# hatoo/rene

Measured on AMD Instinct MI355X. Metric: Mrays/s, higher is better.
Workload: dtype f32

## Files before the change

### include/rene_hip.h

```cpp
#ifndef RENE_HIP_H
#define RENE_HIP_H

#include <stddef.h>
#include <stdint.h>

#ifdef __cplusplus
extern "C" {
#endif

#define RENE_ABI_VERSION 7u

typedef enum rene_status {
  RENE_OK = 0,
  RENE_ERR_INVALID_ARGUMENT = -1,
  RENE_ERR_INVALID_SCENE = -2,
  RENE_ERR_DEVICE = -3,
  RENE_ERR_UNSUPPORTED = -4,
  RENE_ERR_OUT_OF_MEMORY = -5,
  RENE_ERR_IO = -6,
  RENE_ERR_PARSE = -7
} rene_status;


enum { RENE_SHAPE_TRIANGLE = 0, RENE_SHAPE_SPHERE = 1 };
// ... 356 lines not shown

int rene_emitter_pdf(rene_ctx* ctx, size_t n, const float* origins, const float* directions, float* out);

int rene_pcg_probe(int device, uint32_t seed, uint32_t n, uint32_t* out);

int rene_frame_stream_probe(rene_ctx* ctx, uint32_t first_frame, uint32_t n_frames, float* out);

int rene_load_chains(rene_ctx* ctx, const float* chains, size_t n_floats, uint32_t first_frame, uint32_t n_frames,
                     const uint32_t* tile_frames, size_t n_tiles);

#define RENE_COMM_ID_BYTES 128
int rene_comm_unique_id(uint8_t id[RENE_COMM_ID_BYTES]);
int rene_comm_init(rene_ctx* ctx, int n_ranks, int rank, const uint8_t id[RENE_COMM_ID_BYTES]);
int rene_comm_init_all(rene_ctx** ctxs, int n);
int rene_comm_group_begin(void);
int rene_comm_group_end(void);
int rene_reduce(rene_ctx* ctx, int root);
int rene_gather_tiles(rene_ctx* ctx, int root);

void rene_destroy(rene_ctx* ctx);

int rene_scene_pack_info(const rene_scene_desc* scene, rene_pack_info* out);

int rene_plan_memory(const rene_scene_desc* scene, const rene_opts* opts, rene_memory_plan* out);

const char* rene_last_error(void);
uint32_t rene_abi_version(void);


void rene_to_rgb8(const float* sums, size_t n_floats, uint32_t n_samples, uint8_t* out);
void rene_to_aov8(const float* sums, size_t n_floats, uint32_t n_samples, int is_normal, uint8_t* out);
void rene_frame_seeds(uint32_t master_seed, uint32_t first_frame, uint32_t n, uint32_t* out);


typedef struct rene_scene rene_scene;

int rene_scene_load_pbrt(const char* path, rene_scene** out);
int rene_scene_parse_pbrt(const char* text, const char* base_dir, rene_scene** out);
const rene_scene_desc* rene_scene_get_desc(const rene_scene* scene);
const char* rene_scene_film_filename(const rene_scene* scene);
void rene_scene_free(rene_scene* scene);

#ifdef __cplusplus
}
#endif
#endif
// ... 1 lines not shown
```

### rene_amd/abi.py

```python
from __future__ import annotations

import ctypes as C

ABI_VERSION = 7
COMM_ID_BYTES = 128
DEFAULT_SEED = 0x52454E45
TILE_SIZE = 32
FRAME_STREAM_DEPTHS = 50

SHAPE_TRIANGLE, SHAPE_SPHERE = 0, 1
(MATERIAL_NONE, MATERIAL_MATTE, MATERIAL_GLASS, MATERIAL_SUBSTRATE, MATERIAL_METAL,
 MATERIAL_MIRROR, MATERIAL_UBER, MATERIAL_PLASTIC) = range(8)
TEXTURE_SOLID, TEXTURE_CHECKERBOARD, TEXTURE_IMAGEMAP, TEXTURE_SCALE = range(4)
AREA_LIGHT_NULL, AREA_LIGHT_DIFFUSE = 0, 1
LIGHT_DISTANT = 0
INTEGRATOR_PATH, INTEGRATOR_VOLPATH = 0, 1
LAYER_RADIANCE, LAYER_NORMAL, LAYER_ALBEDO = 0, 1, 2
FLAG_COUNTERS, FLAG_NO_AOV, FLAG_FORCE_BVH, FLAG_SINGLE_LEVEL, FLAG_NO_RESTART, FLAG_DYNAMIC_FIRST, FLAG_WAVEFRONT = 1, 2, 4, 8, 16, 32, 64
FLAG_OVERLAP = 128
FLAG_FP16_PAYLOAD = 256
FLAG_FRAME_GROUPS = 1 << 9
FEAT_SMALL = 64
SHARD_TILES, SHARD_FRAMES = 0, 1

STATUS_NAMES = {
    0: "RENE_OK", -1: "RENE_ERR_INVALID_ARGUMENT", -2: "RENE_ERR_INVALID_SCENE",
    -3: "RENE_ERR_DEVICE", -4: "RENE_ERR_UNSUPPORTED", -5: "RENE_ERR_OUT_OF_MEMORY",
    -6: "RENE_ERR_IO", -7: "RENE_ERR_PARSE",
}

f32, u32, i32, u64 = C.c_float, C.c_uint32, C.c_int32, C.c_uint64


class Vertex(C.Structure):
    _fields_ = [("position", f32 * 3), ("normal", f32 * 3), ("uv", f32 * 2)]


class Mesh(C.Structure):
    _fields_ = [("vertices", C.POINTER(Vertex)), ("indices", C.POINTER(u32)),
                ("n_vertices", u32), ("n_indices", u32)]


class Instance(C.Structure):
    _fields_ = [("shape", u32), ("mesh_index", i32), ("material_index", u32),
# ... 167 lines not shown

class Hit(C.Structure):
    _fields_ = [("t", f32), ("u", f32), ("v", f32), ("instance", u32), ("primitive", u32)]


def algorithmic_bytes(stats) -> int:
    g = (lambda k: stats[k]) if isinstance(stats, dict) else (lambda k: getattr(stats, k))
    n_ray = g("rays_closest") + g("rays_shadow") + g("rays_emitter")
    return (64 * n_ray + 64 * g("node_visits") + 48 * g("prim_tests") + 144 * g("hits")
            + 128 * g("bounces") + 32 * g("adds"))


EXPORTED_SYMBOLS = [
    "rene_create", "rene_render", "rene_sync", "rene_download", "rene_reset", "rene_tune", "rene_framebuffer",
    "rene_get_stats", "rene_denoise_params_default", "rene_denoise", "rene_denoise_tiles", "rene_download_denoised", "rene_denoised_buffer",
    "rene_noise_params_default", "rene_estimate_noise", "rene_download_noise_tiles", "rene_noise_combine", "rene_noise_frames_needed",
    "rene_set_active_tiles", "rene_tile_frames", "rene_download_mean", "rene_noise_select_tiles",
    "rene_robust_params_default", "rene_resolve_robust", "rene_download_robust", "rene_download_robust_tiles", "rene_robust_combine",
    "rene_denoise_robust_params_default", "rene_denoise_robust", "rene_denoise_tiles_robust",
    "rene_denoise_shard_bytes", "rene_denoise_shard_prepare", "rene_denoise_shard_buffer", "rene_download_denoise_shard",
    "rene_denoise_place_shard", "rene_denoise_placed", "rene_gather_denoise",
    "rene_feature_params_default", "rene_feature_channels", "rene_export_features", "rene_features_buffer", "rene_download_features", "rene_trace", "rene_ray_dump", "rene_trace_queue", "rene_bsdf_eval", "rene_medium_eval", "rene_emitter_pdf", "rene_pcg_probe", "rene_frame_stream_probe", "rene_load_chains",
    "rene_comm_unique_id", "rene_comm_init", "rene_comm_init_all", "rene_comm_group_begin", "rene_comm_group_end",
    "rene_reduce", "rene_gather_tiles", "rene_destroy", "rene_scene_pack_info", "rene_plan_memory", "rene_last_error", "rene_abi_version",
    "rene_to_rgb8", "rene_to_aov8", "rene_frame_seeds",
    "rene_scene_load_pbrt", "rene_scene_parse_pbrt", "rene_scene_get_desc",
    "rene_scene_film_filename", "rene_scene_free",
]
```

### rene_amd/api.py

```python
from __future__ import annotations

import ctypes as C
import os
import subprocess

import numpy as np

from . import abi

_CSRC = os.path.join(os.path.dirname(os.path.abspath(__file__)), "csrc")
LIB_PATH = os.path.join(_CSRC, os.environ.get("RENE_HIP_LIB", "librene_hip.so"))
_LIB = None


class ReneError(RuntimeError):
    def __init__(self, code: int, message: str):
        super().__init__(f"{abi.STATUS_NAMES.get(code, code)}: {message}")
        self.code = code


def build(force: bool = False) -> str:
    args = ["make", "-C", _CSRC, "-j4"]
    if force:
        args.append("-B")
# ... 60 lines not shown
    L.rene_feature_params_default.argtypes = [C.POINTER(abi.FeatureParams)]
    L.rene_feature_params_default.restype = None
    L.rene_feature_channels.argtypes = [u32]
    L.rene_feature_channels.restype = u32
    L.rene_export_features.argtypes = [vp, C.POINTER(abi.FeatureParams), vp, C.c_size_t]
    L.rene_features_buffer.argtypes = [vp, C.POINTER(vp), C.POINTER(C.c_size_t)]
    L.rene_download_features.argtypes = [vp, vp, C.c_size_t]
    L.rene_trace.argtypes = [vp, i32, C.c_size_t, vp, vp, C.c_float, C.c_float, vp]
    L.rene_bsdf_eval.argtypes = [vp, u32, C.c_size_t, vp, vp, vp, vp, vp, vp]
    L.rene_medium_eval.argtypes = [vp, u32, C.c_size_t, vp, vp, vp, vp, vp, vp]
    L.rene_emitter_pdf.argtypes = [vp, C.c_size_t, vp, vp, vp]
    L.rene_pcg_probe.argtypes = [i32, u32, u32, vp]
    L.rene_frame_stream_probe.argtypes = [vp, u32, u32, vp]
    L.rene_load_chains.argtypes = [vp, vp, C.c_size_t, u32, u32, vp, C.c_size_t]
    L.rene_ray_dump.argtypes = [vp, u32, u32, C.c_size_t, vp, C.POINTER(C.c_uint64)]
    L.rene_trace_queue.argtypes = [vp, C.c_size_t, vp, vp, i32, u32, u32, u32, u32, vp, C.POINTER(C.c_float), vp]
    L.rene_comm_unique_id.argtypes = [vp]
    L.rene_comm_init.argtypes = [vp, i32, i32, vp]
    L.rene_comm_init_all.argtypes = [C.POINTER(vp), i32]
    L.rene_reduce.argtypes = [vp, i32]
    L.rene_gather_tiles.argtypes = [vp, i32]
    L.rene_destroy.argtypes = [vp]
    L.rene_scene_pack_info.argtypes = [C.POINTER(abi.SceneDesc), C.POINTER(abi.PackInfo)]
    L.rene_plan_memory.argtypes = [C.POINTER(abi.SceneDesc), C.POINTER(abi.Opts), C.POINTER(abi.MemoryPlan)]
    L.rene_destroy.restype = None
    L.rene_last_error.restype = C.c_char_p
    L.rene_abi_version.restype = u32
    L.rene_to_rgb8.argtypes = [vp, C.c_size_t, u32, vp]
    L.rene_to_rgb8.restype = None
    L.rene_to_aov8.argtypes = [vp, C.c_size_t, u32, i32, vp]
    L.rene_to_aov8.restype = None
    L.rene_frame_seeds.argtypes = [u32, u32, u32, vp]
    L.rene_frame_seeds.restype = None
    L.rene_scene_load_pbrt.argtypes = [C.c_char_p, C.POINTER(vp)]
    L.rene_scene_parse_pbrt.argtypes = [C.c_char_p, C.c_char_p, C.POINTER(vp)]
    L.rene_scene_get_desc.argtypes = [vp]
    L.rene_scene_get_desc.restype = C.POINTER(abi.SceneDesc)
    L.rene_scene_film_filename.argtypes = [vp]
    L.rene_scene_film_filename.restype = C.c_char_p
    L.rene_scene_free.argtypes = [vp]
    L.rene_scene_free.restype = None
    if L.rene_abi_version() != abi.ABI_VERSION:
        raise ReneError(-1, "librene_hip.so ABI version differs from rene_amd.abi")
    _LIB = L
    return L

# ... 567 lines not shown

Renderer.bsdf_eval = _bsdf_eval


def _medium_eval(self, medium_index: int, rd, t_max, wo, wi, seeds) -> np.ndarray:
    a = [np.ascontiguousarray(v, dtype=np.float32) for v in (rd, t_max, wo, wi)]
    sd = np.ascontiguousarray(seeds, dtype=np.uint32)
    out = np.zeros((sd.size, 16), np.float32)
    p = lambda x: x.ctypes.data_as(C.c_void_p)
    _check(lib().rene_medium_eval(self._h, medium_index, sd.size, p(a[0]), p(a[1]), p(a[2]), p(a[3]), p(sd), p(out)))
    return out


Renderer.medium_eval = _medium_eval


def pack_info(scene) -> abi.PackInfo:
    packed = scene if hasattr(scene, "byref") else scene.to_desc()
    info = abi.PackInfo()
    _check(lib().rene_scene_pack_info(packed.byref(), C.byref(info)))
    return info


def plan_memory(scene, seed: int = abi.DEFAULT_SEED, device: int = 0, flags: int = 0, shard_mode: int = abi.SHARD_TILES,
                shard_rank: int = 0, shard_count: int = 1, framebuffer_ptr: int | None = None, stream_ptr: int | None = None) -> dict:
    packed = scene if hasattr(scene, "byref") else scene.to_desc()
    o = abi.Opts()
    o.struct_size = C.sizeof(abi.Opts)
    o.seed, o.device, o.flags = seed & 0xFFFFFFFF, device, flags
    o.shard_mode, o.shard_rank, o.shard_count = shard_mode, shard_rank, shard_count
    o.framebuffer = framebuffer_ptr
    o.stream = stream_ptr
    plan = abi.MemoryPlan()
    _check(lib().rene_plan_memory(packed.byref(), C.byref(o), C.byref(plan)))
    return plan.as_dict()


def to_rgb8(sums: np.ndarray, n_samples: int) -> np.ndarray:
    a = np.ascontiguousarray(sums, dtype=np.float32)
    out = np.empty(a.shape, dtype=np.uint8)
    lib().rene_to_rgb8(a.ctypes.data_as(C.c_void_p), a.size, n_samples, out.ctypes.data_as(C.c_void_p))
    return out


def to_aov8(sums: np.ndarray, n_samples: int, is_normal: bool) -> np.ndarray:
    a = np.ascontiguousarray(sums, dtype=np.float32)
# ... 10 lines not shown
```

### rene_amd/csrc/device_code.inc

```
#include <hip/hip_runtime.h>

#include <algorithm>
#include <cstdio>
#include <cstdlib>
#include <mutex>
#include <unordered_map>

#include "device_math.h"
#include "device_scene.h"
#include "kernels.h"

namespace rene {

constexpr int BLOCK = 256;

struct HitRec {
  float t, u, v;
  uint32_t slot;
};

struct LaneCounters {
  uint32_t closest = 0, shadow = 0, emitter = 0, paths = 0, hits = 0, adds = 0, nodes = 0, prims = 0;
};

// ... 209 lines not shown
  if (shift == 0u) {
    for (uint32_t i = threadIdx.x; i < P.n_frames; i += BLOCK) T2[i] = frame_seed(P.seed_state0, P.first_frame + i * P.frame_stride);
    return;
  }
  const uint32_t B = 1u << shift, n1 = (P.n_frames + B - 1u) >> shift;
  __attribute__((address_space(3))) uint32_t* T1 = T2 + 2u * B;
  for (uint32_t j = threadIdx.x; j < B; j += BLOCK) {
    uint32_t m, a;
    lcg_pow(j * P.frame_stride, m, a);
    T2[2u * j] = m;
    T2[2u * j + 1u] = a;
  }
  for (uint32_t k = threadIdx.x; k < n1; k += BLOCK) T1[k] = frame_state(P.seed_state0, P.first_frame + (k << shift) * P.frame_stride);
}
RENE_DEV uint32_t launch_seed(const RenderParams& P, const uint32_t* lds_base, uint32_t i) {
  if (P.seed_tab == SEED_TAB_NONE) return frame_seed(P.seed_state0, P.first_frame + i * P.frame_stride);
  const uint32_t shift = P.seed_tab >> 24;
  const __attribute__((address_space(3))) uint32_t* T2 = (const __attribute__((address_space(3))) uint32_t*)lds_base + (P.seed_tab & 0xffffffu);
  if (shift == 0u) return T2[i];
  const uint32_t B = 1u << shift, j = i & (B - 1u);
  return pcg_output(T2[2u * B + (i >> shift)] * T2[2u * j] + T2[2u * j + 1u]);
}

template <bool ANY, bool SPHERES, bool COUNT, bool ITEMS_LDS = false>
RENE_DEV HitRec traverse_small(const Accel& A, const Sphere* spheres, f3 o, f3 d, float tmin, float tmax,
                               LaneCounters& lc, lds_ptr lds_items = nullptr) {
  float best_t = __uint_as_float(__float_as_uint(tmax) + 1u), best_s = 0.0f, best_r = 0.0f;
  uint32_t best_item = 0xffffffffu;
  const uint32_t n = A.n_items;
  typedef const __attribute__((address_space(4))) float16v* item_ptr;
  item_ptr base = (item_ptr)(const void*)A.items;
  auto test_item = [&](const float16v q, const uint32_t k) {
    const float kind = q[12];
    if (COUNT) lc.prims++;
    if (SPHERES && kind == SMALL_KIND_BALL) {
      f3 oc = mk3(o.x - q[0], o.y - q[1], o.z - q[2]);
      float a = length_squared(d);
      float half_b = dot(oc, d);
      float c = length_squared(oc) - q[3];
      float disc = half_b * half_b - a * c;
      if (disc >= 0.0f) {
        float sq = fast_sqrt(disc);
        float inv_a = fast_rcp(a);
        float root0 = (-half_b - sq) * inv_a;
        float root1 = (-half_b + sq) * inv_a;
        float r = -1.0f;
        if (root0 >= tmin && root0 < best_t) r = root0;
        else if (root1 >= tmin && root1 < best_t) r = root1;
        if (r >= tmin && r < best_t) {
          best_t = r;
// ... 44 lines not shown
      }
      const uint32_t open_face = __float_as_uint(q[14]);
      bool use_in = t_in >= tmin, dead = false;
      if (open_face != 0u) {
        const float t_open = open_face == 1u ? t0 : t1;
        use_in = use_in && t_in != t_open;
        dead = !use_in && t_out == t_open;
      }
      const float t = use_in ? t_in : t_out;
      if (t_in <= t_out && !dead && t >= tmin && t < best_t) {
        best_t = t;
        best_item = k;
      }
      return;
    }
    const float n_o = o.x * q[0] + (o.y * q[1] + o.z * q[2]);
    const float n_d = d.x * q[0] + (d.y * q[1] + d.z * q[2]);
    float t = (q[3] - n_o) * __builtin_amdgcn_rcpf(n_d);
    f3 P = mk3(fmaf(t, d.x, o.x), fmaf(t, d.y, o.y), fmaf(t, d.z, o.z));
    const float sr_x = fmaf(P.x, q[4], fmaf(P.y, q[6], P.z * q[8])) + q[10];
    const float sr_y = fmaf(P.x, q[5], fmaf(P.y, q[7], P.z * q[9])) + q[11];
    const float lim_x = fmaf(-kind, sr_y, 1.0f - sr_x), lim_y = fmaf(-kind, sr_x, 1.0f - sr_y);
    bool accept = fminf(fminf(sr_x, sr_y), fminf(lim_x, lim_y)) >= 0.0f && t >= tmin && t < best_t;
    if (accept) {
      best_t = t;
      best_s = sr_x;
      best_r = sr_y;
      best_item = k;
    }
  };
  for (uint32_t k = 0; k < n; ++k) test_item(base[k], k);
  HitRec h;
  h.t = best_t;
  h.u = 0.0f;
  h.v = 0.0f;
  h.slot = 0xffffffffu;
  if (ANY && best_item != 0xffffffffu) {
    h.slot = 0u;
    return h;
  }
  if (best_item != 0xffffffffu) {
    float4 m = ITEMS_LDS ? lds4(lds_items + 16u * best_item + 12u) : ldg4(A.items[best_item].q + 12);
    if (m.x == SMALL_KIND_BOX) {
      float4 b0, b1, b2;
      if (ITEMS_LDS) {
        lds_ptr bq = lds_items + 16u * best_item;
// ... 885 lines not shown
template <bool SPHERES>
RENE_DEV float emitter_pdf_lds(const SceneView& S, const SmallLds& T, const HitRec& h, f3 ro, f3 rd) {
  if (h.slot == 0xffffffffu) return 0.0f;
  lds_ptr q = T.emit + SMALL_EMIT_FLOATS * h.slot;
  const float4 a = lds4(q), b = lds4(q + 4), c = lds4(q + 8), pr = lds4(q + 12);
  const float primitive_count = q[16];
  uint32_t sidx = __float_as_uint(c.w);
  if (SPHERES && sidx != 0xffffffffu) {
    const lds_ptr sq = T.spheres + 24u * sidx;
    const float4 m0 = lds4(sq), m1 = lds4(sq + 4), m2 = lds4(sq + 8);
    const float m[12] = {m0.x, m0.y, m0.z, m0.w, m1.x, m1.y, m1.z, m1.w, m2.x, m2.y, m2.z, m2.w};
    float radius = (fabsf(m[0]) + fabsf(m[4]) + fabsf(m[8])) / 3.0f;
    f3 center = mk3(m[9], m[10], m[11]);
    float cos_theta_max = fast_sqrt(fmaxf(1.0f - qdiv(radius * radius, length_squared(center - ro)), 0.0f));
    float solid_angle = 2.0f * kPi * (1.0f - cos_theta_max);
    return fast_rcp(solid_angle);
  }
  f3 p0 = mk3(a.x, a.y, a.z), e1 = mk3(a.w, b.x, b.y), e2 = mk3(b.z, b.w, c.x);
  f3 hit_pos = p0 + h.u * e1 + h.v * e2;
  float distance_squared = length_squared(ro - hit_pos);
  float cosine = fabsf(dot(normalize(rd), mk3(pr.x, pr.y, pr.z)));
  return qdiv(qdiv(distance_squared, cosine * pr.w), primitive_count);
}
template <bool SPHERES>
RENE_DEV f3 emit_sample_lds(const SmallLds& T, uint32_t obj, Pcg& rng) {
  lds_ptr e = T.eobj + 16u * obj;
  const float4 head = lds4(e);
  if (SPHERES && __float_as_uint(head.x) == 1u) {
    f3 v = normalize(random_in_unit_sphere(rng));
    const float4 m0 = lds4(e + 4), m1 = lds4(e + 8), m2 = lds4(e + 12);
    const float m[12] = {m0.x, m0.y, m0.z, m0.w, m1.x, m1.y, m1.z, m1.w, m2.x, m2.y, m2.z, m2.w};
    return aff_point(m, v);
  }
  uint32_t p = umod(pcg_u32(rng), __float_as_uint(head.z));
  lds_ptr q = T.etri + 12u * (__float_as_uint(head.y) + p);
  const float4 a = lds4(q), b = lds4(q + 4), c = lds4(q + 8);
  float r = pcg_f32(rng);
  float s = pcg_f32(rng);
  if (r + s > 1.0f) {
    r = 1.0f - r;
    s = 1.0f - s;
  }
  return mk3(a.x, a.y, a.z) * (1.0f - r - s) + mk3(a.w, b.x, b.y) * r + mk3(b.z, b.w, c.x) * s;
}

struct MediumRec {
// ... 383 lines not shown
  V.shade = global_ptr<PrimShade>(karg_u64_at<RENE_SKARG(shade)>(KB, tick));
  V.emit_pdf = global_ptr<EmitPdf>(karg_u64_at<RENE_SKARG(emit_pdf)>(KB, tick));
  V.insts = global_ptr<Inst>(karg_u64_at<RENE_SKARG(insts)>(KB, tick));
  V.emit_objects = global_ptr<EmitObject>(karg_u64_at<RENE_SKARG(emit_objects)>(KB, tick));
  V.emit_tris = global_ptr<EmitTri>(karg_u64_at<RENE_SKARG(emit_tris)>(KB, tick));
  V.materials = global_ptr<Material>(karg_u64_at<RENE_SKARG(materials)>(KB, tick));
  V.textures = global_ptr<Texture>(karg_u64_at<RENE_SKARG(textures)>(KB, tick));
  V.lights = global_ptr<Light>(karg_u64_at<RENE_SKARG(lights)>(KB, tick));
  V.images = global_ptr<ImageRef>(karg_u64_at<RENE_SKARG(images)>(KB, tick));
  V.image_pool = global_ptr<float>(karg_u64_at<RENE_SKARG(image_pool)>(KB, tick));
  V.uni = global_ptr<struct Uniforms>(karg_u64_at<RENE_SKARG(uni)>(KB, tick));
  return V;
}

#ifdef RENE_NO_FRAME_STREAM_TABLE
constexpr bool kFrameStreamTable = false;
#else
constexpr bool kFrameStreamTable = true;
#endif
#ifndef RENE_FRAME_STREAM_LOAD_EARLY
#define RENE_FRAME_STREAM_LOAD_EARLY 0
#endif
constexpr bool frame_stream_feat(uint32_t feat) { return kFrameStreamTable && (feat & FEAT_SMALL) && !(feat & (FEAT_VOLPATH | FEAT_SPHERES)) && lobe_kinds(feat) == 0; }
RENE_DEV float4 frame_stream_load(const float* table, uint32_t launch_frame, uint32_t depth) {
  const uint32_t off = ((launch_frame << FRAME_STREAM_STRIDE_LOG2) + depth) << 4;
  const lds_v4 e = *(const __attribute__((address_space(1))) lds_v4*)((const __attribute__((address_space(1))) char*)table + off);
  return make_float4(e.x, e.y, e.z, e.w);
}
template <bool SPHERES>
RENE_DEV void frame_stream_row(const SceneView& S, uint32_t seed, float4* row) {
  Pcg fw = pcg_new(seed);
  for (uint32_t depth = 0; depth < FRAME_STREAM_DEPTHS; ++depth) {
    f3 on_light = splat(0.0f);
    uint32_t light = 0u;
    if (S.emit_object_len > 0) {
      if (pcg_f32(fw) > 0.5f) {
        uint32_t obj = umod(pcg_u32(fw), S.emit_object_len);
        on_light = emit_sample<SPHERES>(S, obj, fw);
        light = 0x80000000u;
      }
    }
    float rr_coin = 0.0f;
    if (depth > 12) rr_coin = pcg_f32(fw);
    row[depth] = make_float4(on_light.x, on_light.y, on_light.z, __uint_as_float(__float_as_uint(rr_coin) | light));
  }
}

#ifndef RENE_REGEN_MIN
#define RENE_REGEN_MIN 1
#endif
template <uint32_t FEAT, int MAXL, bool COUNT, bool AOV>
#ifndef RENE_SMALL_GEN1_PLAIN_WAVES
#define RENE_SMALL_GEN1_PLAIN_WAVES 1
#endif
#ifndef RENE_SMALL_GEN1_WAVES
#define RENE_SMALL_GEN1_WAVES 1
#endif
__global__ void __launch_bounds__(BLOCK, (FEAT & FEAT_SMALL) && !(FEAT & FEAT_VOLPATH) ? (!(FEAT & FEAT_GENERAL_BSDF) ? RENE_SMALL_MATTE_WAVES : (MAXL == 1 ? ((FEAT & FEAT_TEXTURES) ? RENE_SMALL_GEN1_WAVES : RENE_SMALL_GEN1_PLAIN_WAVES) : 1)) : 1) render_kernel(SceneView S, RenderParams P) {
  constexpr bool SPHERES = (FEAT & FEAT_SPHERES) != 0;
  constexpr uint32_t GENERAL = lobe_kinds(FEAT);
  constexpr bool SMALL = (FEAT & FEAT_SMALL) != 0;
  constexpr bool VOL = (FEAT & FEAT_VOLPATH) != 0;
  extern __shared__ uint32_t s_stack[];
  uint32_t* stack = s_stack + threadIdx.x;
  constexpr bool LDS = SMALL && !VOL;
  constexpr bool FWTAB = frame_stream_feat(FEAT);
  SmallLds T{};
  if constexpr (LDS) {
    small_lds_fill(S, s_stack);
    T = small_lds(S, s_stack);
  }
  seed_tables_fill(P, s_stack);
  __syncthreads();

  LaneCounters lc;
  const uint32_t W = S.width, H = S.height;
  const float tmin = 0.001f, tmax = 100000.0f;

  uint32_t ver = 0, pxy = 0, frame = 0, frame_end = 0;
  const karg_ptr KB = (karg_ptr)__builtin_amdgcn_kernarg_segment_ptr();
  auto rec_offset = [&]() { return pixel_record(KB, pxy & 0x3fffu, H - 1 - ((pxy >> 14) & 0x3fffu), pxy >> 28) * 4; };
  bool waiting = false;
  f3 acc0 = splat(0.0f), acc1 = splat(0.0f), acc2 = splat(0.0f);
  bool active = false, done = false;
  f3 ro = splat(0.0f), rd = splat(0.0f), color = splat(0.0f);
  Pcg rng{0}, fw{0};
  int depth = 0;
  uint32_t medium_index = 0;

  const size_t layer_stride = (size_t)(P.n_work >> CHAINS_LOG2) * 4;
  uint32_t batch_next = 0, batch_ll = 0;
  bool exhausted = false;
  first_batch(P, KB, batch_next, batch_ll);
  clock_probe(P, false);

  uint32_t iter = 0;
  uint32_t ln_active = 0, ln_wait = 0, ln_idle = 0, ln_start = 0, st_switch = 0, st_poll = 0;
  for (;; ++iter) {
    bool finished = !active && !waiting && ver != 0u && frame == frame_end;
    if (finished) {
      float* p = reinterpret_cast<float*>(karg_u64<RENE_KARG(framebuffer)>(KB)) + rec_offset();
      item_commit<AOV>(ver, p, layer_stride, acc0, acc1, acc2);
      ver = 0u;
    }
    if (COUNT && __any(finished)) st_switch++;
    bool need = !done && ver == 0u;
    bool fresh = false;
    if (__any(need)) {
      if ((batch_ll & 0xffffu) == 0u && !exhausted) exhausted = !batch_refill(KB, batch_next, batch_ll);
      unsigned long long mask = __ballot(need);
      uint32_t rank = (uint32_t)__popcll(mask & ((1ull << lane_id()) - 1ull));
// ... 62 lines not shown
      if (n_start < RENE_REGEN_MIN && __any(active)) start_now = false;
    }
    if (start_now) {
      const uint32_t seed = launch_seed(P, s_stack, frame);
      frame += CHAINS;
      const uint32_t px = pxy & 0x3fffu, py = (pxy >> 14) & 0x3fffu;
      rng = pcg_new((py * W + px) ^ seed);
      if constexpr (!FWTAB) fw = pcg_new(seed);
      float u = qdiv((float)px + pcg_f32(rng), (float)(W - 1));
      float v = qdiv((float)py + pcg_f32(rng), (float)(H - 1));
      cfloat_ptr cam = (cfloat_ptr)(const void*)S.uni;
      f3 origin = camera_origin(cam);
      f3 target = m4_point(cam + 16, mk3(u * 2.0f - 1.0f, v * 2.0f - 1.0f, 1.0f));
      target = m4_point(cam, target);
      ro = origin;
      rd = normalize(target - origin);
      color = splat(1.0f);
      depth = 0;
      medium_index = 0;
      active = true;
    }

    if (active) {
      lc.closest++;
      float4 fwe = make_float4(0.0f, 0.0f, 0.0f, 0.0f);
      if constexpr (FWTAB && RENE_FRAME_STREAM_LOAD_EARLY) fwe = frame_stream_load(P.frame_stream, frame - CHAINS, (uint32_t)depth);
      HitRec h = trace_accel<SMALL, false, SPHERES, COUNT, LDS>(S.main, S.spheres, ro, rd, tmin, tmax, stack, lc, T.items_main);
      if (h.slot == 0xffffffffu) {
        f3 bg = splat(0.0f);
        if (FEAT & FEAT_BACKGROUND) {
          uv2 uv = sphere_uv(normalize(m4_vector(S.uni->bg_matrix, rd)));
          bg = mk3(S.uni->bg_color[0], S.uni->bg_color[1], S.uni->bg_color[2]) * background_tex<FEAT>(S, uv);
        }
        acc0 = acc0 + color * bg;
        lc.adds++;
        active = false;
      } else if (VOL) {
        lc.hits++;
        Surface sf = shade_hit<SPHERES>(S, h, ro, rd);
        const Inst& inst = S.insts[sf.instance];
        f3 wo = -normalize(rd);
        f3 normal = normalize(sf.normal);
        f3 position = sf.position;
        MediumRec medium = load_medium(S, medium_index);
        bool scattered = false;
        if (medium.type != RENE_MEDIUM_VACUUM) {
          SampledMedium sm = medium_sample(medium, ro, rd, h.t, rng);
          color = color * sm.tr;
          scattered = sm.sampled;
          if (scattered) ro = sm.position;
        }
// ... 121 lines not shown
        }
        if (depth == 0) {
          if (AOV) {
            acc1 = acc1 + normal;
            acc2 = acc2 + material_albedo<FEAT>(L, inst, sf.uv);
          }
          lc.adds += 2;
        }
        if (FEAT & FEAT_LIGHTS) {
          for (uint32_t li = 0; li < L.lights_len; ++li) {
            float4 ld = ldg4(L.lights[li].dir), lL = ldg4(L.lights[li].L);
            f3 target = position + mk3(ld.x, ld.y, ld.z);
            f3 wi = normalize(target - position);
            lc.shadow++;
            HitRec sh = trace_accel<SMALL, true, SPHERES, COUNT, LDS>(S.main, S.spheres, position, wi, tmin, 1e5f, stack, lc, T.items_main);
            if (sh.slot == 0xffffffffu) {
              f3 f = bsdf_f<MAXL, GENERAL>(bsdf, wo, wi);
              acc0 = acc0 + color * f * fabsf(dot(wi, normal)) * mk3(lL.x, lL.y, lL.z);
              lc.adds++;
            }
          }
        }
        bool alive = true;
        if (L.emit_object_len > 0 && bsdf_contains<MAXL, GENERAL>(bsdf, K_DIFFUSE)) {
          f3 wi, f;
          float pdf;
          bool pick_light;
          if constexpr (FWTAB) pick_light = (__float_as_uint(fwe.w) >> 31) != 0u;
          else pick_light = pcg_f32(fw) > 0.5f;
          if (pick_light) {
            f3 on_light;
            if constexpr (FWTAB) {
              on_light = mk3(fwe.x, fwe.y, fwe.z);
            } else {
              uint32_t obj = umod(pcg_u32(fw), L.emit_object_len);
              if constexpr (LDS) on_light = emit_sample_lds<SPHERES>(T, obj, fw);
              else on_light = emit_sample<SPHERES>(L, obj, fw);
            }
            wi = normalize(on_light - position);
            pdf = bsdf_pdf<MAXL, GENERAL>(bsdf, wi, normal);
            f = bsdf_f<MAXL, GENERAL>(bsdf, wo, wi);
          } else {
            Sampled s = bsdf_sample<MAXL, GENERAL>(bsdf, wo, rng);
            wi = s.wi;
            pdf = s.pdf;
            f = s.f;
          }
          ro = position;
          rd = wi;
          lc.emitter++;
          HitRec eh = trace_accel<SMALL, false, SPHERES, COUNT, LDS>(S.emit, S.spheres, ro, rd, tmin, tmax, stack, lc, T.items_emit);
          float pdf_l;
          if constexpr (LDS) pdf_l = emitter_pdf_lds<SPHERES>(L, T, eh, ro, rd);
          else pdf_l = emitter_pdf<SPHERES>(L, eh, ro, rd);
          color = color * (f * fabsf(dot(normal, wi)));
          pdf = 0.5f * pdf + qdiv(0.5f * pdf_l, (float)L.emit_object_len);
          if (pdf < 1e-5f) alive = false;
          else color = color / pdf;
        } else {
          Sampled s = bsdf_sample<MAXL, GENERAL>(bsdf, wo, rng);
          if (s.pdf < 1e-5f) {
            alive = false;
          } else {
            color = color * (s.f * qdiv(fabsf(dot(normal, s.wi)), s.pdf));
            ro = position;
            rd = s.wi;
          }
        }
        if (alive && is_zero(color)) alive = false;
        if (alive && depth > 12) {
          float rr_coin;
          if constexpr (FWTAB) rr_coin = fabsf(fwe.w);
          else rr_coin = pcg_f32(fw);
          float continue_p = max_element(color);
          if (rr_coin > continue_p) alive = false;
          else color = color / continue_p;
        }
        depth++;
        if (depth >= 50) alive = false;
        active = alive;
      }
    }
  }

  clock_probe(P, true);
  unsigned long long sums[8] = {wave_sum(lc.closest), wave_sum(lc.shadow), wave_sum(lc.emitter),
                                wave_sum(lc.paths),   wave_sum(lc.hits),   wave_sum(lc.adds),
                                wave_sum(lc.nodes),   wave_sum(lc.prims)};
  if (lane_id() == 0) {
#pragma unroll
    for (int i = 0; i < 8; ++i)
      if (sums[i]) atomicAdd(&P.counters[i], sums[i]);
  }
  if (COUNT) {
    unsigned long long a = wave_sum(ln_active), b = wave_sum(ln_wait), c = wave_sum(ln_idle), d = wave_sum(ln_start);
    if (lane_id() == 0) {
      atomicAdd(&P.counters[12], (unsigned long long)iter);
      atomicAdd(&P.counters[13], a);
      atomicAdd(&P.counters[14], b);
// ... 18 lines not shown
```

### rene_amd/csrc/device_scene.h

```cpp
#pragma once
#include <stdint.h>

namespace rene {

struct Node {
  float q[16];
};
constexpr uint32_t TOP_NODES_MAX = 341;
constexpr uint32_t LEAF_BIT = 0x80000000u;
constexpr uint32_t SPHERE_BIT = 0x40000000u;
constexpr uint32_t LEAF_COUNT_SHIFT = 26;
constexpr uint32_t LEAF_FIRST_MASK = (1u << 26) - 1u;
constexpr uint32_t MAX_LEAF_PRIMS = 16;

struct PrimIsect {
  float q[12];
};

struct PrimShade {
  float q[16];
};

struct EmitPdf {
  float q[4];
// ... 41 lines not shown
struct Texture {
  uint32_t type;
  uint32_t u0[4];
  float v0[4];
  uint32_t pad[3];
};
struct Light {
  float dir[4];
  float L[4];
};
struct ImageRef {
  uint64_t offset;
  uint32_t width, height;
};
struct Medium {
  float sa_g[4];
  float ss_t[4];
};
struct InstMedium {
  uint32_t interior;
  uint32_t exterior;
};

struct SmallItem {
  float q[16];
};
constexpr uint32_t SMALL_MAX_ITEMS = 64;
constexpr float SMALL_KIND_QUAD = 0.0f, SMALL_KIND_TRIANGLE = 1.0f, SMALL_KIND_SPHERE = 2.0f, SMALL_KIND_BOX = 3.0f,
                SMALL_KIND_BALL = 4.0f;

constexpr uint32_t SMALL_LDS_MAX_BYTES = 22u * 1024u;
enum : uint32_t { SMALL_OFF_EMIT_ITEMS = 0, SMALL_OFF_HIT, SMALL_OFF_EMIT, SMALL_OFF_EOBJ, SMALL_OFF_ETRI, SMALL_OFF_SPHERES, SMALL_OFF_COUNT };
constexpr uint32_t SMALL_HIT_FLOATS = 52, SMALL_EMIT_FLOATS = 20;

struct Accel {
  const Node* nodes;
  const PrimIsect* isect;
  const SmallItem* items;
  uint32_t n_nodes;
  uint32_t n_slots;
  uint32_t n_items;
  uint32_t n_top;
};

struct Uniforms {
  float c2w[16];
// ... 120 lines not shown
```

### rene_amd/csrc/rene_hip.cpp

```cpp
#include "../../include/rene_hip.h"

#include <hip/hip_runtime.h>
#include <dlfcn.h>
#include <rccl/rccl.h>

#include <algorithm>
#include <chrono>
#include <thread>
#include <cmath>
#include <cstdio>
#include <cstdlib>
#include <cstring>
#include <deque>
#include <functional>
#include <memory>
#include <optional>
#include <string>
#include <vector>

#include "device_scene.h"
#include "kernels.h"
#include "launch_plan.h"
#include "scene_pack.h"

// ... 750 lines not shown
  out->n_spheres = (uint32_t)ps.spheres.size();
  out->n_nodes_main = (uint32_t)ps.main.nodes.size();
  out->n_slots_main = (uint32_t)ps.main.isect.size();
  out->depth_main = ps.main.depth;
  out->n_nodes_emit = (uint32_t)ps.emit.nodes.size();
  out->n_slots_emit = (uint32_t)ps.emit.isect.size();
  out->depth_emit = ps.emit.depth;
  out->features = ps.features;
  out->emit_object_len = (uint32_t)ps.emit_objects.size();
  out->lights_len = (uint32_t)ps.lights.size();
  out->n_items_main = (ps.features & rene::FEAT_SMALL) ? ps.main.n_loop : 0u;
  out->n_items_emit = (ps.features & rene::FEAT_SMALL) ? ps.emit.n_loop : 0u;
  out->device_bytes = ps.main.nodes.size() * sizeof(rene::Node) + ps.main.isect.size() * sizeof(rene::PrimIsect) +
                      ps.emit.nodes.size() * sizeof(rene::Node) + ps.emit.isect.size() * sizeof(rene::PrimIsect) +
                      ps.shade.size() * sizeof(rene::PrimShade) + ps.emit_pdf.size() * sizeof(rene::EmitPdf) +
                      ps.spheres.size() * sizeof(rene::Sphere) + ps.insts.size() * sizeof(rene::Inst) +
                      ps.emit_objects.size() * sizeof(rene::EmitObject) + ps.emit_tris.size() * sizeof(rene::EmitTri) +
                      ps.materials.size() * sizeof(rene::Material) + ps.textures.size() * sizeof(rene::Texture) +
                      ps.lights.size() * sizeof(rene::Light) + ps.image_pool.size() * sizeof(float) +
                      ps.mediums.size() * sizeof(rene::Medium) + ps.inst_medium.size() * sizeof(rene::InstMedium);
  return RENE_OK;
}

namespace {
struct ContextPlan {
  rene_memory_plan bytes{};
  uint32_t tiles_x = 0, n_tiles = 0, n_slots = 0, features = 0, depth = 0, stack = 0;
  uint64_t owned_pixels = 0;
  bool wavefront = false;
  static constexpr uint32_t kWaveMaxLights = 4;
  static constexpr int kQueues = 11;
  size_t queue[kQueues] = {};
};
}
static size_t fixed_bytes() { return rene_ctx::kCounters * sizeof(uint32_t) + 32 * sizeof(unsigned long long); }
static int read_opts(const rene_opts* opts, rene_opts& o) {
  o = rene_opts{};
  o.struct_size = sizeof(rene_opts);
  o.seed = RENE_DEFAULT_SEED;
  if (opts) {
    if (opts->struct_size != sizeof(rene_opts))
      return fail(RENE_ERR_INVALID_ARGUMENT, "rene_opts.struct_size mismatch (ABI skew)");
    o = *opts;
  }
  if (o.shard_count == 0) o.shard_count = 1;
  if (o.shard_rank >= o.shard_count) return fail(RENE_ERR_INVALID_ARGUMENT, "shard_rank >= shard_count");
// ... 1877 lines not shown
static uint8_t sat_u8(float v) {
  if (!(v > 0.0f)) return 0;
  if (v >= 255.0f) return 255;
  return (uint8_t)v;
}
void rene_to_rgb8(const float* sums, size_t n_floats, uint32_t n_samples, uint8_t* out) {
  const float denom = (float)n_samples;
  for (size_t i = 0; i < n_floats; ++i) {
    float v = sums[i] / denom;
    float r = std::round(255.0f * gamma_correct(v));
    out[i] = sat_u8(std::fmin(std::fmax(r, 0.0f), 255.0f));
  }
}
void rene_to_aov8(const float* sums, size_t n_floats, uint32_t n_samples, int is_normal, uint8_t* out) {
  const float denom = (float)n_samples;
  for (size_t i = 0; i < n_floats; ++i) {
    float v = sums[i] / denom;
    if (is_normal) v = v * 0.5f + 0.5f;
    out[i] = sat_u8(256.0f * std::fmin(std::fmax(v, 0.0f), 0.999f));
  }
}

int rene_scene_pack_info(const rene_scene_desc* scene, rene_pack_info* out) { return guarded([&] { return rene_scene_pack_info_impl(scene, out); }); }
int rene_plan_memory(const rene_scene_desc* scene, const rene_opts* opts, rene_memory_plan* out) { return guarded([&] { return rene_plan_memory_impl(scene, opts, out); }); }
int rene_create(const rene_scene_desc* scene, const rene_opts* opts, rene_ctx** out) { return guarded([&] { return rene_create_impl(scene, opts, out); }); }
int rene_render(rene_ctx* c, uint32_t first_frame, uint32_t n_frames) { return guarded([&] { return rene_render_impl(c, first_frame, n_frames); }); }
int rene_download(rene_ctx* c, int layer, int channels, float* dst, size_t dst_floats) { return guarded([&] { return rene_download_impl(c, layer, channels, dst, dst_floats); }); }
int rene_estimate_noise(rene_ctx* c, const rene_noise_params* params, rene_noise_estimate* out) { return guarded([&] { return rene_estimate_noise_impl(c, params, out); }); }
int rene_set_active_tiles(rene_ctx* c, const uint8_t* active, size_t n) { return guarded([&] { return rene_set_active_tiles_impl(c, active, n); }); }
int rene_tile_frames(rene_ctx* c, uint32_t* dst, size_t n) { return guarded([&] { return rene_tile_frames_impl(c, dst, n); }); }
int rene_download_mean(rene_ctx* c, int layer, int channels, float* dst, size_t dst_floats) { return guarded([&] { return rene_download_mean_impl(c, layer, channels, dst, dst_floats); }); }
int rene_noise_select_tiles(const rene_noise_tile* tiles, const uint8_t* active_in, uint32_t tiles_x, uint32_t tiles_y, float luminance_floor, double target, uint32_t dilate,
                            uint8_t* active_out) {
  return guarded([&] { return rene_noise_select_tiles_impl(tiles, active_in, tiles_x, tiles_y, luminance_floor, target, dilate, active_out); });
}
int rene_download_noise_tiles(rene_ctx* c, rene_noise_tile* dst, size_t n) { return guarded([&] { return rene_download_noise_tiles_impl(c, dst, n); }); }
int rene_resolve_robust(rene_ctx* c, const rene_robust_params* params, rene_robust_summary* out) { return guarded([&] { return rene_resolve_robust_impl(c, params, out); }); }
int rene_download_robust(rene_ctx* c, int what, int channels, float* dst, size_t dst_floats) { return guarded([&] { return rene_download_robust_impl(c, what, channels, dst, dst_floats); }); }
int rene_export_features(rene_ctx* c, const rene_feature_params* params, void* device_dst, size_t dst_bytes) { return guarded([&] { return rene_export_features_impl(c, params, device_dst, dst_bytes); }); }
int rene_features_buffer(rene_ctx* c, void** device_ptr, size_t* n_bytes) { return guarded([&] { return rene_features_buffer_impl(c, device_ptr, n_bytes); }); }
int rene_download_features(rene_ctx* c, void* dst, size_t dst_bytes) { return guarded([&] { return rene_download_features_impl(c, dst, dst_bytes); }); }
int rene_download_robust_tiles(rene_ctx* c, rene_robust_tile* dst, size_t n) { return guarded([&] { return rene_download_robust_tiles_impl(c, dst, n); }); }
int rene_load_chains(rene_ctx* c, const float* chains, size_t n_floats, uint32_t first_frame, uint32_t n_frames, const uint32_t* tile_frames, size_t n_tiles) {
  return guarded([&] { return rene_load_chains_impl(c, chains, n_floats, first_frame, n_frames, tile_frames, n_tiles); });
}
int rene_denoise_shard_prepare(rene_ctx* c, const rene_denoise_params* params) { return guarded([&] { return rene_denoise_shard_prepare_impl(c, params); }); }
// ... 5 lines not shown
```

### rene_amd/csrc/scene_pack.cpp

```cpp
#include "scene_pack.h"

#include <algorithm>
#include <cmath>
#include <cstdlib>
#include <cstring>
#include <limits>

namespace rene {
namespace {

struct V3 {
  float x, y, z;
};
inline V3 sub(V3 a, V3 b) { return {a.x - b.x, a.y - b.y, a.z - b.z}; }
inline V3 cross(V3 a, V3 b) {
  return {a.y * b.z - a.z * b.y, a.z * b.x - a.x * b.z, a.x * b.y - a.y * b.x};
}
inline float dot(V3 a, V3 b) { return a.x * b.x + a.y * b.y + a.z * b.z; }

struct Box {
  float lo[3], hi[3];
  void reset() {
    for (int a = 0; a < 3; ++a) {
      lo[a] = std::numeric_limits<float>::infinity();
// ... 550 lines not shown
    }
    if (!boxes.empty()) {
      std::vector<SmallItem> items;
      std::sort(boxes.begin(), boxes.end(), [](const Box6& x, const Box6& y) { return x.first < y.first; });
      for (size_t i = 0; i < n_items; ++i) {
        for (const Box6& bx : boxes)
          if (bx.first == i) items.push_back(bx.item);
        if (!gone[i]) items.push_back(acc.items[i]);
      }
      const size_t n_loop = items.size();
      size_t nb = 0;
      for (SmallItem& it : items)
        if (it.q[12] == SMALL_KIND_BOX) it.q[13] = bits_to_float((uint32_t)(n_loop + nb++));
      for (const Box6& bx : boxes) items.push_back(bx.aux);
      acc.items = std::move(items);
      acc.n_loop = (uint32_t)n_loop;
    } else {
      acc.n_loop = (uint32_t)acc.items.size();
    }
  }
  if (acc.n_loop > SMALL_MAX_ITEMS || acc.isect.size() > 255) { acc.items.clear(); acc.n_loop = 0; }
}

void finish_accel(const std::vector<Prim>& prims, uint32_t max_leaf, BuiltAccel& out,
                  std::vector<uint32_t>& order) {
  Builder b(prims, max_leaf);
  b.build();
  Collapse4 wide(b.nodes);
  out.depth = wide.run();
  out.nodes = std::move(wide.out);
  {
    const size_t n = out.nodes.size();
    std::vector<uint32_t> fresh(n, 0xffffffffu), bfs;
    std::vector<uint32_t> level{0u};
    auto inner_children = [&](uint32_t i, std::vector<uint32_t>& to) {
      for (int c = 0; c < 4; ++c) {
        const uint32_t w = float_bits(out.nodes[i].q[4 + c]);
        if (!(w & LEAF_BIT)) to.push_back(w);
      }
    };
    while (!level.empty() && bfs.size() + level.size() <= TOP_NODES_MAX) {
      std::vector<uint32_t> next;
      for (uint32_t i : level) {
        fresh[i] = (uint32_t)bfs.size();
        bfs.push_back(i);
        inner_children(i, next);
// ... 312 lines not shown
          et.q[5] = pw[1].z; et.q[6] = pw[2].x; et.q[7] = pw[2].y; et.q[8] = pw[2].z;
          out.emit_tris.push_back(et);
        }
      }
      out.n_triangles += ntri;
    } else {
      err = "unknown instance shape";
      return RENE_ERR_INVALID_SCENE;
    }
    out.insts.push_back(inst);
  }
  if (prims.size() > LEAF_FIRST_MASK) { err = "too many primitives for the 26-bit leaf index"; return RENE_ERR_UNSUPPORTED; }
  if (out.emit_objects.empty()) out.features |= FEAT_NO_EMITTERS;

  std::vector<uint32_t> order;
  uint32_t max_leaf = 2;
  if (const char* e = std::getenv("RENE_MAX_LEAF")) max_leaf = (uint32_t)std::max(1, std::min(16, std::atoi(e)));
  finish_accel(prims, max_leaf, out.main, order);
  out.shade.resize(prims.size());
  for (size_t s = 0; s < prims.size(); ++s) out.shade[s] = prims[order[s]].shade;
  finish_accel(eprims, max_leaf, out.emit, order);
  out.emit_pdf.resize(eprims.size());
  for (size_t s = 0; s < eprims.size(); ++s) out.emit_pdf[s] = eprims[order[s]].pdf;
  if (!out.main.items.empty() && (eprims.empty() || !out.emit.items.empty())) {
    std::vector<float>& img = out.small_image;
    auto append = [&](const float* p, size_t n) { img.insert(img.end(), p, p + n); };
    auto bits = [](float f) { uint32_t u; std::memcpy(&u, &f, 4); return u; };
    for (const SmallItem& it : out.main.items) append(it.q, 16);
    out.small_off[SMALL_OFF_EMIT_ITEMS] = (uint32_t)(img.size() * 4);
    for (const SmallItem& it : out.emit.items) append(it.q, 16);
    out.small_off[SMALL_OFF_HIT] = (uint32_t)(img.size() * 4);
    for (size_t s = 0; s < out.main.isect.size(); ++s) {
      append(out.main.isect[s].q, 12);
      append(out.shade[s].q, 16);
      const Inst& in = out.insts[bits(out.main.isect[s].q[9])];
      static_assert(sizeof(Inst) == 96 && SMALL_HIT_FLOATS == 12 + 16 + 24, "Inst is six float4");
      append(reinterpret_cast<const float*>(&in), 24);
    }
    out.small_off[SMALL_OFF_EMIT] = (uint32_t)(img.size() * 4);
    for (size_t s = 0; s < out.emit.isect.size(); ++s) {
      append(out.emit.isect[s].q, 12);
      append(out.emit_pdf[s].q, 4);
      const float tail[4] = {out.insts[bits(out.emit.isect[s].q[9])].primitive_count, 0.f, 0.f, 0.f};
      append(tail, 4);
    }
    out.small_off[SMALL_OFF_EOBJ] = (uint32_t)(img.size() * 4);
// ... 15 lines not shown
```

Baseline: 139,200.

## Fuse emitter MIS trace into next closest-hit traversal via marked emitter twin item

When the emitter accel holds a single quad or triangle that also appears exactly once in the main small item list, that main item is flagged as an emit twin. The next bounce's closest-hit traversal then records whether the ray hits the twin unoccluded, and the emitter pdf, MIS weighting and Russian roulette are deferred to that point. This removes the separate emitter-BVH trace per diffuse bounce. In exchange it adds state carried across iterations, duplicated roulette logic and adjusted counters, with some risk to correctness on edge cases. It also adds an API to export the small items.

```diff
diff --git a/include/rene_hip.h b/include/rene_hip.h
--- a/include/rene_hip.h
+++ b/include/rene_hip.h
@@ -402,6 +402,8 @@
 
 int rene_scene_pack_info(const rene_scene_desc* scene, rene_pack_info* out);
 
+int rene_scene_small_items(const rene_scene_desc* scene, int which, float* out, uint32_t cap_items, uint32_t* n_loop, uint32_t* n_total);
+
 int rene_plan_memory(const rene_scene_desc* scene, const rene_opts* opts, rene_memory_plan* out);
 
 const char* rene_last_error(void);
diff --git a/rene_amd/abi.py b/rene_amd/abi.py
--- a/rene_amd/abi.py
+++ b/rene_amd/abi.py
@@ -20,6 +20,7 @@
 FLAG_OVERLAP = 128
 FLAG_FP16_PAYLOAD = 256
 FLAG_FRAME_GROUPS = 1 << 9
+SMALL_ITEM_EMIT_TWIN = 0x80000000
 FEAT_SMALL = 64
 SHARD_TILES, SHARD_FRAMES = 0, 1
 
@@ -233,7 +234,7 @@
     "rene_denoise_place_shard", "rene_denoise_placed", "rene_gather_denoise",
     "rene_feature_params_default", "rene_feature_channels", "rene_export_features", "rene_features_buffer", "rene_download_features", "rene_trace", "rene_ray_dump", "rene_trace_queue", "rene_bsdf_eval", "rene_medium_eval", "rene_emitter_pdf", "rene_pcg_probe", "rene_frame_stream_probe", "rene_load_chains",
     "rene_comm_unique_id", "rene_comm_init", "rene_comm_init_all", "rene_comm_group_begin", "rene_comm_group_end",
-    "rene_reduce", "rene_gather_tiles", "rene_destroy", "rene_scene_pack_info", "rene_plan_memory", "rene_last_error", "rene_abi_version",
+    "rene_reduce", "rene_gather_tiles", "rene_destroy", "rene_scene_pack_info", "rene_scene_small_items", "rene_plan_memory", "rene_last_error", "rene_abi_version",
     "rene_to_rgb8", "rene_to_aov8", "rene_frame_seeds",
     "rene_scene_load_pbrt", "rene_scene_parse_pbrt", "rene_scene_get_desc",
     "rene_scene_film_filename", "rene_scene_free",
diff --git a/rene_amd/api.py b/rene_amd/api.py
--- a/rene_amd/api.py
+++ b/rene_amd/api.py
@@ -106,6 +106,7 @@
     L.rene_gather_tiles.argtypes = [vp, i32]
     L.rene_destroy.argtypes = [vp]
     L.rene_scene_pack_info.argtypes = [C.POINTER(abi.SceneDesc), C.POINTER(abi.PackInfo)]
+    L.rene_scene_small_items.argtypes = [C.POINTER(abi.SceneDesc), C.c_int, vp, u32, C.POINTER(u32), C.POINTER(u32)]
     L.rene_plan_memory.argtypes = [C.POINTER(abi.SceneDesc), C.POINTER(abi.Opts), C.POINTER(abi.MemoryPlan)]
     L.rene_destroy.restype = None
     L.rene_last_error.restype = C.c_char_p
@@ -719,6 +720,16 @@
     return info
 
 
+def small_items(scene, which: int = 0):
+    packed = scene if hasattr(scene, "byref") else scene.to_desc()
+    n_loop, n_total = C.c_uint32(0), C.c_uint32(0)
+    _check(lib().rene_scene_small_items(packed.byref(), which, None, 0, C.byref(n_loop), C.byref(n_total)))
+    out = np.zeros((n_total.value, 16), np.uint32)
+    if n_total.value:
+        _check(lib().rene_scene_small_items(packed.byref(), which, out.ctypes.data_as(C.c_void_p), n_total.value, C.byref(n_loop), None))
+    return out, n_loop.value
+
+
 def plan_memory(scene, seed: int = abi.DEFAULT_SEED, device: int = 0, flags: int = 0, shard_mode: int = abi.SHARD_TILES,
                 shard_rank: int = 0, shard_count: int = 1, framebuffer_ptr: int | None = None, stream_ptr: int | None = None) -> dict:
     packed = scene if hasattr(scene, "byref") else scene.to_desc()
diff --git a/rene_amd/csrc/device_code.inc b/rene_amd/csrc/device_code.inc
--- a/rene_amd/csrc/device_code.inc
+++ b/rene_amd/csrc/device_code.inc
@@ -255,10 +255,15 @@
   return pcg_output(T2[2u * B + (i >> shift)] * T2[2u * j] + T2[2u * j + 1u]);
 }
 
-template <bool ANY, bool SPHERES, bool COUNT, bool ITEMS_LDS = false>
+struct EmitCapture {
+  float s = -1.0f, r = 0.0f;
+  uint32_t seen = 0u;
+};
+template <bool ANY, bool SPHERES, bool COUNT, bool ITEMS_LDS = false, bool CAPTURE = false>
 RENE_DEV HitRec traverse_small(const Accel& A, const Sphere* spheres, f3 o, f3 d, float tmin, float tmax,
-                               LaneCounters& lc, lds_ptr lds_items = nullptr) {
-  float best_t = __uint_as_float(__float_as_uint(tmax) + 1u), best_s = 0.0f, best_r = 0.0f;
+                               LaneCounters& lc, lds_ptr lds_items = nullptr, EmitCapture* cap = nullptr) {
+  const float first_t = __uint_as_float(__float_as_uint(tmax) + 1u);
+  float best_t = first_t, best_s = 0.0f, best_r = 0.0f;
   uint32_t best_item = 0xffffffffu;
   const uint32_t n = A.n_items;
   typedef const __attribute__((address_space(4))) float16v* item_ptr;
@@ -349,6 +354,14 @@
     const float sr_y = fmaf(P.x, q[5], fmaf(P.y, q[7], P.z * q[9])) + q[11];
     const float lim_x = fmaf(-kind, sr_y, 1.0f - sr_x), lim_y = fmaf(-kind, sr_x, 1.0f - sr_y);
     bool accept = fminf(fminf(sr_x, sr_y), fminf(lim_x, lim_y)) >= 0.0f && t >= tmin && t < best_t;
+    if constexpr (CAPTURE) {
+      if (__float_as_uint(q[15]) & SMALL_ITEM_EMIT_TWIN) {
+        const bool alone = fminf(fminf(sr_x, sr_y), fminf(lim_x, lim_y)) >= 0.0f && t >= tmin && t < first_t;
+        cap->s = alone ? sr_x : -1.0f;
+        cap->r = sr_y;
+        cap->seen = 1u;
+      }
+    }
     if (accept) {
       best_t = t;
       best_s = sr_x;
@@ -1280,6 +1293,27 @@
   float cosine = fabsf(dot(normalize(rd), mk3(pr.x, pr.y, pr.z)));
   return qdiv(qdiv(distance_squared, cosine * pr.w), primitive_count);
 }
+RENE_DEV HitRec emit_twin_hit(const SmallLds& T, const EmitCapture& cap, float tmax) {
+  HitRec h;
+  h.t = tmax;
+  h.u = 0.0f;
+  h.v = 0.0f;
+  h.slot = 0xffffffffu;
+  if (cap.s != -1.0f) {
+    const float4 m = lds4(T.items_emit + 12u);
+    const float best_s = cap.s, best_r = cap.r;
+    bool second = m.x == SMALL_KIND_QUAD && best_s + best_r > 1.0f;
+    uint32_t perm = __float_as_uint(m.w) >> (second ? 8u : 0u);
+    float w0 = second ? best_s + best_r - 1.0f : 1.0f - best_s - best_r;
+    float w1 = second ? 1.0f - best_r : best_s;
+    float w2 = second ? 1.0f - best_s : best_r;
+    uint32_t iu = perm & 3u, iv = (perm >> 2) & 3u;
+    h.u = iu == 0u ? w0 : (iu == 1u ? w1 : w2);
+    h.v = iv == 0u ? w0 : (iv == 1u ? w1 : w2);
+    h.slot = __float_as_uint(second ? m.z : m.y);
+  }
+  return h;
+}
 template <bool SPHERES>
 RENE_DEV f3 emit_sample_lds(const SmallLds& T, uint32_t obj, Pcg& rng) {
   lds_ptr e = T.eobj + 16u * obj;
@@ -1709,6 +1743,12 @@
 #define RENE_FRAME_STREAM_LOAD_EARLY 0
 #endif
 constexpr bool frame_stream_feat(uint32_t feat) { return kFrameStreamTable && (feat & FEAT_SMALL) && !(feat & (FEAT_VOLPATH | FEAT_SPHERES)) && lobe_kinds(feat) == 0; }
+#ifdef RENE_NO_EMIT_FUSION
+constexpr bool kEmitFusion = false;
+#else
+constexpr bool kEmitFusion = true;
+#endif
+constexpr bool emit_fusion_feat(uint32_t feat) { return kEmitFusion && frame_stream_feat(feat); }
 RENE_DEV float4 frame_stream_load(const float* table, uint32_t launch_frame, uint32_t depth) {
   const uint32_t off = ((launch_frame << FRAME_STREAM_STRIDE_LOG2) + depth) << 4;
   const lds_v4 e = *(const __attribute__((address_space(1))) lds_v4*)((const __attribute__((address_space(1))) char*)table + off);
@@ -1752,6 +1792,7 @@
   uint32_t* stack = s_stack + threadIdx.x;
   constexpr bool LDS = SMALL && !VOL;
   constexpr bool FWTAB = frame_stream_feat(FEAT);
+  constexpr bool EFUSE = emit_fusion_feat(FEAT);
   SmallLds T{};
   if constexpr (LDS) {
     small_lds_fill(S, s_stack);
@@ -1774,6 +1815,7 @@
   Pcg rng{0}, fw{0};
   int depth = 0;
   uint32_t medium_index = 0;
+  [[maybe_unused]] float pdf_bsdf = 0.0f;
 
   const size_t layer_stride = (size_t)(P.n_work >> CHAINS_LOG2) * 4;
   uint32_t batch_next = 0, batch_ll = 0;
@@ -1882,11 +1924,37 @@
     }
 
     if (active) {
-      lc.closest++;
+      if constexpr (!EFUSE) lc.closest++;
       float4 fwe = make_float4(0.0f, 0.0f, 0.0f, 0.0f);
       if constexpr (FWTAB && RENE_FRAME_STREAM_LOAD_EARLY) fwe = frame_stream_load(P.frame_stream, frame - CHAINS, (uint32_t)depth);
-      HitRec h = trace_accel<SMALL, false, SPHERES, COUNT, LDS>(S.main, S.spheres, ro, rd, tmin, tmax, stack, lc, T.items_main);
-      if (h.slot == 0xffffffffu) {
+      HitRec h;
+      [[maybe_unused]] EmitCapture cap;
+      if constexpr (EFUSE) {
+        h = traverse_small<false, SPHERES, COUNT, LDS, true>(S.main, S.spheres, ro, rd, tmin, tmax, lc, T.items_main, &cap);
+        if (cap.seen != 0u && depth > 0) {
+          const HitRec eh = emit_twin_hit(T, cap, tmax);
+          const float pdf_l = emitter_pdf_lds<SPHERES>(S, T, eh, ro, rd);
+          float pdf = pdf_bsdf;
+          bool alive = true;
+          pdf = 0.5f * pdf + qdiv(0.5f * pdf_l, (float)S.emit_object_len);
+          if (pdf < 1e-5f) alive = false;
+          else color = color / pdf;
+          if (alive && is_zero(color)) alive = false;
+          if (alive && depth - 1 > 12) {
+            const float rr_coin = fabsf(frame_stream_load(P.frame_stream, frame - CHAINS, (uint32_t)(depth - 1)).w);
+            float continue_p = max_element(color);
+            if (rr_coin > continue_p) alive = false;
+            else color = color / continue_p;
+          }
+          if (COUNT && !alive) lc.prims -= S.main.n_items;
+          active = alive;
+        }
+        if (active) lc.closest++;
+      } else {
+        h = trace_accel<SMALL, false, SPHERES, COUNT, LDS>(S.main, S.spheres, ro, rd, tmin, tmax, stack, lc, T.items_main);
+      }
+      if (EFUSE && !active) {
+      } else if (h.slot == 0xffffffffu) {
         f3 bg = splat(0.0f);
         if (FEAT & FEAT_BACKGROUND) {
           uv2 uv = sphere_uv(normalize(m4_vector(S.uni->bg_matrix, rd)));
@@ -2054,6 +2122,7 @@
           }
         }
         bool alive = true;
+        [[maybe_unused]] bool deferred = false;
         if (L.emit_object_len > 0 && bsdf_contains<MAXL, GENERAL>(bsdf, K_DIFFUSE)) {
           f3 wi, f;
           float pdf;
@@ -2081,14 +2150,22 @@
           ro = position;
           rd = wi;
           lc.emitter++;
-          HitRec eh = trace_accel<SMALL, false, SPHERES, COUNT, LDS>(S.emit, S.spheres, ro, rd, tmin, tmax, stack, lc, T.items_emit);
-          float pdf_l;
-          if constexpr (LDS) pdf_l = emitter_pdf_lds<SPHERES>(L, T, eh, ro, rd);
-          else pdf_l = emitter_pdf<SPHERES>(L, eh, ro, rd);
-          color = color * (f * fabsf(dot(normal, wi)));
-          pdf = 0.5f * pdf + qdiv(0.5f * pdf_l, (float)L.emit_object_len);
-          if (pdf < 1e-5f) alive = false;
-          else color = color / pdf;
+          if (EFUSE && cap.seen != 0u) {
+            if (COUNT) lc.prims++;
+            color = color * (f * fabsf(dot(normal, wi)));
+            pdf_bsdf = pdf;
+            deferred = true;
+            if (is_zero(color) && pdf == pdf && length_squared(ro) < __builtin_inff()) alive = false;
+          } else {
+            HitRec eh = trace_accel<SMALL, false, SPHERES, COUNT, LDS>(S.emit, S.spheres, ro, rd, tmin, tmax, stack, lc, T.items_emit);
+            float pdf_l;
+            if constexpr (LDS) pdf_l = emitter_pdf_lds<SPHERES>(L, T, eh, ro, rd);
+            else pdf_l = emitter_pdf<SPHERES>(L, eh, ro, rd);
+            color = color * (f * fabsf(dot(normal, wi)));
+            pdf = 0.5f * pdf + qdiv(0.5f * pdf_l, (float)L.emit_object_len);
+            if (pdf < 1e-5f) alive = false;
+            else color = color / pdf;
+          }
         } else {
           Sampled s = bsdf_sample<MAXL, GENERAL>(bsdf, wo, rng);
           if (s.pdf < 1e-5f) {
@@ -2099,14 +2176,16 @@
             rd = s.wi;
           }
         }
-        if (alive && is_zero(color)) alive = false;
-        if (alive && depth > 12) {
-          float rr_coin;
-          if constexpr (FWTAB) rr_coin = fabsf(fwe.w);
-          else rr_coin = pcg_f32(fw);
-          float continue_p = max_element(color);
-          if (rr_coin > continue_p) alive = false;
-          else color = color / continue_p;
+        if (!(EFUSE && deferred)) {
+          if (alive && is_zero(color)) alive = false;
+          if (alive && depth > 12) {
+            float rr_coin;
+            if constexpr (FWTAB) rr_coin = fabsf(fwe.w);
+            else rr_coin = pcg_f32(fw);
+            float continue_p = max_element(color);
+            if (rr_coin > continue_p) alive = false;
+            else color = color / continue_p;
+          }
         }
         depth++;
         if (depth >= 50) alive = false;
diff --git a/rene_amd/csrc/device_scene.h b/rene_amd/csrc/device_scene.h
--- a/rene_amd/csrc/device_scene.h
+++ b/rene_amd/csrc/device_scene.h
@@ -87,6 +87,7 @@
   uint32_t exterior;
 };
 
+constexpr uint32_t SMALL_ITEM_EMIT_TWIN = 0x80000000u;
 struct SmallItem {
   float q[16];
 };
diff --git a/rene_amd/csrc/rene_hip.cpp b/rene_amd/csrc/rene_hip.cpp
--- a/rene_amd/csrc/rene_hip.cpp
+++ b/rene_amd/csrc/rene_hip.cpp
@@ -796,6 +796,23 @@
   return RENE_OK;
 }
 
+static int rene_scene_small_items_impl(const rene_scene_desc* scene, int which, float* out, uint32_t cap_items, uint32_t* n_loop, uint32_t* n_total) {
+  if (!scene || !n_loop || (cap_items && !out)) return fail(RENE_ERR_INVALID_ARGUMENT, "rene_scene_small_items: NULL argument");
+  if (which != 0 && which != 1) return fail(RENE_ERR_INVALID_ARGUMENT, "rene_scene_small_items: which must be 0 (main) or 1 (emitter)");
+  rene::PackedScene ps;
+  std::string err;
+  int rc = rene::pack_scene(scene, ps, err);
+  if (rc != RENE_OK) return fail(rc, err);
+  const rene::BuiltAccel& acc = which == 0 ? ps.main : ps.emit;
+  const bool small = (ps.features & rene::FEAT_SMALL) != 0;
+  const size_t n = small ? acc.items.size() : 0;
+  *n_loop = small ? acc.n_loop : 0u;
+  if (n_total) *n_total = (uint32_t)n;
+  const size_t take = std::min<size_t>(n, cap_items);
+  if (take) std::memcpy(out, acc.items.data(), take * sizeof(rene::SmallItem));
+  return RENE_OK;
+}
+
 namespace {
 struct ContextPlan {
   rene_memory_plan bytes{};
@@ -2719,6 +2736,9 @@
 }
 
 int rene_scene_pack_info(const rene_scene_desc* scene, rene_pack_info* out) { return guarded([&] { return rene_scene_pack_info_impl(scene, out); }); }
+int rene_scene_small_items(const rene_scene_desc* scene, int which, float* out, uint32_t cap_items, uint32_t* n_loop, uint32_t* n_total) {
+  return guarded([&] { return rene_scene_small_items_impl(scene, which, out, cap_items, n_loop, n_total); });
+}
 int rene_plan_memory(const rene_scene_desc* scene, const rene_opts* opts, rene_memory_plan* out) { return guarded([&] { return rene_plan_memory_impl(scene, opts, out); }); }
 int rene_create(const rene_scene_desc* scene, const rene_opts* opts, rene_ctx** out) { return guarded([&] { return rene_create_impl(scene, opts, out); }); }
 int rene_render(rene_ctx* c, uint32_t first_frame, uint32_t n_frames) { return guarded([&] { return rene_render_impl(c, first_frame, n_frames); }); }
diff --git a/rene_amd/csrc/scene_pack.cpp b/rene_amd/csrc/scene_pack.cpp
--- a/rene_amd/csrc/scene_pack.cpp
+++ b/rene_amd/csrc/scene_pack.cpp
@@ -596,6 +596,29 @@
   if (acc.n_loop > SMALL_MAX_ITEMS || acc.isect.size() > 255) { acc.items.clear(); acc.n_loop = 0; }
 }
 
+void mark_emit_twin(BuiltAccel& main, const BuiltAccel& emit) {
+#ifdef RENE_NO_EMIT_FUSION
+  (void)main; (void)emit;
+#else
+  if (const char* e = std::getenv("RENE_EMIT_FUSION"))
+    if (std::atoi(e) == 0) return;
+  if (emit.n_loop != 1 || emit.items.size() != 1 || main.items.empty()) return;
+  const SmallItem& em = emit.items[0];
+  if (em.q[12] != SMALL_KIND_QUAD && em.q[12] != SMALL_KIND_TRIANGLE) return;
+  if (em.q[0] == 0.0f && em.q[1] == 0.0f && em.q[2] == 0.0f) return;
+  int twin = -1, twins = 0;
+  for (uint32_t i = 0; i < main.n_loop; ++i) {
+    const SmallItem& it = main.items[i];
+    if (std::memcmp(it.q, em.q, 13 * sizeof(float)) == 0 && (float_bits(it.q[15]) & 0xffffu) == (float_bits(em.q[15]) & 0xffffu)) {
+      twin = (int)i;
+      twins++;
+    }
+  }
+  if (twins != 1) return;
+  main.items[twin].q[15] = bits_to_float(float_bits(main.items[twin].q[15]) | SMALL_ITEM_EMIT_TWIN);
+#endif
+}
+
 void finish_accel(const std::vector<Prim>& prims, uint32_t max_leaf, BuiltAccel& out,
                   std::vector<uint32_t>& order) {
   Builder b(prims, max_leaf);
@@ -954,6 +977,7 @@
   finish_accel(eprims, max_leaf, out.emit, order);
   out.emit_pdf.resize(eprims.size());
   for (size_t s = 0; s < eprims.size(); ++s) out.emit_pdf[s] = eprims[order[s]].pdf;
+  mark_emit_twin(out.main, out.emit);
   if (!out.main.items.empty() && (eprims.empty() || !out.emit.items.empty())) {
     std::vector<float>& img = out.small_image;
     auto append = [&](const float* p, size_t n) { img.insert(img.end(), p, p + n); };
```

Result: faster. 141,100 (median of 6 runs) (+1.4%).
